# andabi/parallel-wavenet-vocoder

Hardware: AMD Instinct MI355X
Metric: audio samples/sec, 4-flow IAF generation (higher is better)
Workload: dtype f32 via 3-term split-fp16 MFMA (fp32 accumulate, fp32 storage)

## Files before the change

### parallel-wavenet-vocoder_amd/csrc/pwv_misc.hip

```cpp
#include "pwv_common.h"

#include <cstring>

namespace pwv {

static thread_local char g_err[512] = {0};
char* error_buffer() { return g_err; }
int set_error(int code, const char* fmt, ...) {
    va_list ap;
    va_start(ap, fmt);
    vsnprintf(g_err, sizeof(g_err), fmt, ap);
    va_end(ap);
    return code;
}

__global__ void causal_conv_kernel(const float* __restrict__ x, const float* __restrict__ f, float* __restrict__ y,
                                   int N, int T, int Cin, int Cout, int W, int d) {
    const int co4 = (Cout + 3) / 4;
    const long long idx = (long long)blockIdx.x * blockDim.x + threadIdx.x;
    const long long total = (long long)N * T * co4;
    if (idx >= total) return;
    const int c4 = (int)(idx % co4);
    const long long row = idx / co4;
    const int t = (int)(row % T);
// ... 56 lines not shown
        const int m = rt * 32 + j;
        const bool mvalid = m < M;
        const int mc = mvalid ? m : M - 1;
        float xb[KH4 * 4];
        const float* xr = x + (size_t)mc * K + h * kh;
        bool keep = true;
        if (conv_T > 0) {
            keep = h == 1 || (mc % conv_T) >= conv_d;
            xr = x + (size_t)(mc - ((h == 0 && keep) ? conv_d : 0)) * kh;
        }
#pragma unroll
        for (int g = 0; g < KH4; ++g) {
            f32x4 v = {0.f, 0.f, 0.f, 0.f};
            if (4 * g < kh && keep) v = *reinterpret_cast<const f32x4*>(xr + 4 * g);
#pragma unroll
            for (int e = 0; e < 4; ++e) xb[4 * g + e] = v[e];
        }
        f32x16 acc[4];
#pragma unroll
        for (int it = 0; it < 4; ++it)
#pragma unroll
            for (int r = 0; r < 16; ++r) {
                const int n = n0 + chan_of(it, r, h);
                acc[it][r] = (bias && n < Nout) ? bias[n] : 0.f;
            }
        f32x4 a[4];
#pragma unroll
        for (int it = 0; it < 4; ++it) a[it] = *reinterpret_cast<const f32x4*>(&lds[((it * KH4) * 64 + lane) * 4]);
#pragma unroll
        for (int g = 0; g < KH4; ++g) {
            if (4 * g < kh) {
                f32x4 nx[4] = {a[0], a[1], a[2], a[3]};
                if (g + 1 < KH4) {
#pragma unroll
                    for (int it = 0; it < 4; ++it)
                        nx[it] = *reinterpret_cast<const f32x4*>(&lds[((it * KH4 + g + 1) * 64 + lane) * 4]);
                }
                __builtin_amdgcn_sched_barrier(0);
#pragma unroll
                for (int e = 0; e < 4; ++e)
#pragma unroll
                    for (int it = 0; it < 4; ++it)
                        acc[it] = __builtin_amdgcn_mfma_f32_32x32x2f32(a[it][e], xb[4 * g + e], acc[it], 0, 0, 0);
                __builtin_amdgcn_sched_barrier(0);
#pragma unroll
                for (int it = 0; it < 4; ++it) a[it] = nx[it];
            }
        }
        if (mvalid) {
#pragma unroll
            for (int it = 0; it < 4; ++it)
#pragma unroll
                for (int q = 0; q < 4; ++q) {
                    const int n = n0 + 32 * it + 8 * q + 4 * h;
                    if (n < Nout) {
                        f32x4 v = {acc[it][q * 4], acc[it][q * 4 + 1], acc[it][q * 4 + 2], acc[it][q * 4 + 3]};
                        if (relu) {
#pragma unroll
                            for (int e = 0; e < 4; ++e) v[e] = fmaxf(v[e], 0.f);
                        }
                        *reinterpret_cast<f32x4*>(y + (size_t)m * Nout + n) = v;
                    }
                }
        }
    }
}

typedef float f32x2m __attribute__((ext_vector_type(2)));
__device__ __forceinline__ void split8m(const float (&x)[8], f16x8& hi, f16x8& lo) {
#pragma unroll
    for (int q = 0; q < 8; q += 2) {
        const f32x2m v = {x[q], x[q + 1]};
        const f16x2 h = __builtin_convertvector(v, f16x2);
        const f32x2m r = v - __builtin_convertvector(h, f32x2m);
        const f16x2 l = __builtin_convertvector(r, f16x2);
        hi[q] = h[0];
        hi[q + 1] = h[1];
        lo[q] = l[0];
        lo[q + 1] = l[1];
    }
}

template <int NS>
__global__ __launch_bounds__(256) void linear_split_kernel(const float* __restrict__ x, const float* __restrict__ w,
                                                           const float* __restrict__ bias, float* __restrict__ y, int M,
                                                           int K, int Nout, int relu) {
    __shared__ __attribute__((aligned(16))) f16x8 lds[2 * 4 * NS * 64];
    const int tid = threadIdx.x;
    const int lane = tid & 63;
    const int wave = __builtin_amdgcn_readfirstlane(tid >> 6);
    const int h = lane >> 5, j = lane & 31;
    const int n0 = blockIdx.y * 128;
    for (int item = tid; item < 128 * NS * 2; item += 256) {
        const int c = item & 127, sh = item >> 7, ss = sh >> 1, hh = sh & 1;
        float v[8];
#pragma unroll
        for (int q = 0; q < 8; ++q) {
            const int k = 16 * ss + 8 * hh + q;
            v[q] = (k < K && n0 + c < Nout) ? w[(size_t)k * Nout + n0 + c] : 0.f;
        }
        f16x8 hi, lo;
        split8m(v, hi, lo);
        const int unit = ((c >> 5) * NS + ss) * 64 + hh * 32 + (c & 31);
        lds[unit] = hi;
        lds[4 * NS * 64 + unit] = lo;
    }
    __syncthreads();
    const f16x8* AH = lds;
    const f16x8* AL = lds + 4 * NS * 64;
    const int row_tiles = (M + 31) / 32;
    for (int rt = blockIdx.x * 4 + wave; rt < row_tiles; rt += gridDim.x * 4) {
        const int m = rt * 32 + j;
        const bool mvalid = m < M;
        const int mc = mvalid ? m : M - 1;
        f16x8 bh[NS], bl[NS];
#pragma unroll
        for (int ss = 0; ss < NS; ++ss) {
            float v[8];
#pragma unroll
            for (int g = 0; g < 2; ++g) {
                const int k = 16 * ss + 8 * h + 4 * g;
                f32x4 t = {0.f, 0.f, 0.f, 0.f};
                if (k < K) t = *reinterpret_cast<const f32x4*>(x + (size_t)mc * K + k);
#pragma unroll
                for (int e = 0; e < 4; ++e) v[4 * g + e] = t[e];
            }
            split8m(v, bh[ss], bl[ss]);
        }
        f32x16 acc[4];
#pragma unroll
        for (int it = 0; it < 4; ++it) {
            const int n = n0 + 32 * it + j;
            const float bv = (bias && n < Nout) ? bias[n] : 0.f;
#pragma unroll
            for (int r = 0; r < 16; ++r) acc[it][r] = bv;
        }
#pragma unroll
        for (int ss = 0; ss < NS; ++ss) {
            f16x8 ah[4], al[4];
#pragma unroll
            for (int it = 0; it < 4; ++it) {
                ah[it] = AH[(it * NS + ss) * 64 + lane];
                al[it] = AL[(it * NS + ss) * 64 + lane];
            }
#pragma unroll
            for (int it = 0; it < 4; ++it) {
                acc[it] = __builtin_amdgcn_mfma_f32_32x32x16_f16(bh[ss], ah[it], acc[it], 0, 0, 0);
                acc[it] = __builtin_amdgcn_mfma_f32_32x32x16_f16(bl[ss], ah[it], acc[it], 0, 0, 0);
                acc[it] = __builtin_amdgcn_mfma_f32_32x32x16_f16(bh[ss], al[it], acc[it], 0, 0, 0);
            }
        }
#pragma unroll
        for (int it = 0; it < 4; ++it) {
            const int n = n0 + 32 * it + j;
#pragma unroll
            for (int r = 0; r < 16; ++r) {
                const int mr = rt * 32 + 8 * (r >> 2) + 4 * h + (r & 3);
                float v = acc[it][r];
                if (relu) v = fmaxf(v, 0.f);
                if (mr < M && n < Nout) __hip_atomic_store(&y[(size_t)mr * Nout + n], v, __ATOMIC_RELAXED, __HIP_MEMORY_SCOPE_AGENT);
            }
        }
    }
}

constexpr int kCtStride = 84;
__global__ __launch_bounds__(256) void cond_proj_kernel(const float* __restrict__ x0, const float* __restrict__ w0, int K0,
                                                        const float* __restrict__ w, const float* __restrict__ bias, float* __restrict__ y,
                                                        float* __restrict__ frames, int M, int K, int Nout, float limit, int* flag) {
    constexpr int NS = 5;
    __shared__ __attribute__((aligned(16))) f16x8 lds[2 * 4 * NS * 64];
    __shared__ __attribute__((aligned(16))) f16x8 lds0[2 * 4 * NS * 64];
    __shared__ __attribute__((aligned(16))) float ct[4][32 * kCtStride];
    const int tid = threadIdx.x;
    const int lane = tid & 63;
    const int wave = __builtin_amdgcn_readfirstlane(tid >> 6);
    const int h = lane >> 5, j = lane & 31;
    const int n0 = blockIdx.y * 128;
    for (int item = tid; item < 128 * NS * 2; item += 256) {
        const int c = item & 127, sh = item >> 7, ss = sh >> 1, hh = sh & 1;
        float v[8], v0[8];
#pragma unroll
        for (int q = 0; q < 8; ++q) {
            const int k = 16 * ss + 8 * hh + q;
            v[q] = (k < K && n0 + c < Nout) ? w[(size_t)k * Nout + n0 + c] : 0.f;
            v0[q] = (k < K0 && c < K) ? w0[(size_t)k * K + c] : 0.f;
        }
        f16x8 hi, lo;
        split8m(v, hi, lo);
        const int unit = ((c >> 5) * NS + ss) * 64 + hh * 32 + (c & 31);
        lds[unit] = hi;
        lds[4 * NS * 64 + unit] = lo;
        split8m(v0, hi, lo);
        lds0[unit] = hi;
        lds0[4 * NS * 64 + unit] = lo;
    }
    __syncthreads();
    const f16x8* AH = lds;
    const f16x8* AL = lds + 4 * NS * 64;
    const f16x8* A0H = lds0;
    const f16x8* A0L = lds0 + 4 * NS * 64;
    float* const ctw = ct[wave];
    const int row_tiles = (M + 31) / 32;
    for (int rt = blockIdx.x * 4 + wave; rt < row_tiles; rt += gridDim.x * 4) {
        const int m = rt * 32 + j;
        const bool mvalid = m < M;
        const int mc = mvalid ? m : M - 1;
        f16x8 bh[NS], bl[NS];
        bool bad = false;
#pragma unroll
        for (int ss = 0; ss < NS; ++ss) {
            float v[8];
#pragma unroll
            for (int g = 0; g < 2; ++g) {
                const int k = 16 * ss + 8 * h + 4 * g;
                f32x4 t = {0.f, 0.f, 0.f, 0.f};
                if (k < K0) t = *reinterpret_cast<const f32x4*>(x0 + (size_t)mc * K0 + k);
#pragma unroll
                for (int e = 0; e < 4; ++e) {
                    v[4 * g + e] = t[e];
                    bad = bad || !(fabsf(t[e]) <= limit);
                }
            }
            split8m(v, bh[ss], bl[ss]);
        }
        if (flag && bad) __hip_atomic_store(flag, 1, __ATOMIC_RELAXED, __HIP_MEMORY_SCOPE_SYSTEM);
        f32x16 acc0[3];
#pragma unroll
        for (int it = 0; it < 3; ++it)
#pragma unroll
            for (int r = 0; r < 16; ++r) acc0[it][r] = 0.f;
#pragma unroll
        for (int ss = 0; ss < NS; ++ss) {
            f16x8 ah[3], al[3];
#pragma unroll
            for (int it = 0; it < 3; ++it) {
                ah[it] = A0H[(it * NS + ss) * 64 + lane];
                al[it] = A0L[(it * NS + ss) * 64 + lane];
            }
#pragma unroll
            for (int it = 0; it < 3; ++it) {
                acc0[it] = __builtin_amdgcn_mfma_f32_32x32x16_f16(bh[ss], ah[it], acc0[it], 0, 0, 0);
                acc0[it] = __builtin_amdgcn_mfma_f32_32x32x16_f16(bl[ss], ah[it], acc0[it], 0, 0, 0);
                acc0[it] = __builtin_amdgcn_mfma_f32_32x32x16_f16(bh[ss], al[it], acc0[it], 0, 0, 0);
            }
        }
#pragma unroll
        for (int it = 0; it < 3; ++it) {
            const int n = 32 * it + j;
#pragma unroll
            for (int r = 0; r < 16; ++r) {
                const int ml = 8 * (r >> 2) + 4 * h + (r & 3);
                const float v = fmaxf(acc0[it][r], 0.f);
                if (n < K) {
                    ctw[ml * kCtStride + n] = v;
                    const int mr = rt * 32 + ml;
                    if (frames && blockIdx.y == 0 && mr < M) __hip_atomic_store(&frames[(size_t)mr * K + n], v, __ATOMIC_RELAXED, __HIP_MEMORY_SCOPE_AGENT);
                }
            }
        }
        asm volatile("s_waitcnt lgkmcnt(0)" ::: "memory");
#pragma unroll
        for (int ss = 0; ss < NS; ++ss) {
            float v[8];
#pragma unroll
            for (int g = 0; g < 2; ++g) {
                const int k = 16 * ss + 8 * h + 4 * g;
                f32x4 t = {0.f, 0.f, 0.f, 0.f};
                if (k < K) t = *reinterpret_cast<const f32x4*>(&ctw[j * kCtStride + k]);
#pragma unroll
                for (int e = 0; e < 4; ++e) v[4 * g + e] = t[e];
            }
            split8m(v, bh[ss], bl[ss]);
        }
        asm volatile("s_waitcnt lgkmcnt(0)" ::: "memory");
        f32x16 acc[4];
#pragma unroll
        for (int it = 0; it < 4; ++it) {
            const int n = n0 + 32 * it + j;
            const float bv = (bias && n < Nout) ? bias[n] : 0.f;
#pragma unroll
            for (int r = 0; r < 16; ++r) acc[it][r] = bv;
        }
#pragma unroll
        for (int ss = 0; ss < NS; ++ss) {
            f16x8 ah[4], al[4];
#pragma unroll
            for (int it = 0; it < 4; ++it) {
                ah[it] = AH[(it * NS + ss) * 64 + lane];
                al[it] = AL[(it * NS + ss) * 64 + lane];
            }
#pragma unroll
            for (int it = 0; it < 4; ++it) {
                acc[it] = __builtin_amdgcn_mfma_f32_32x32x16_f16(bh[ss], ah[it], acc[it], 0, 0, 0);
                acc[it] = __builtin_amdgcn_mfma_f32_32x32x16_f16(bl[ss], ah[it], acc[it], 0, 0, 0);
                acc[it] = __builtin_amdgcn_mfma_f32_32x32x16_f16(bh[ss], al[it], acc[it], 0, 0, 0);
            }
        }
#pragma unroll
        for (int it = 0; it < 4; ++it) {
            const int n = n0 + 32 * it + j;
#pragma unroll
            for (int r = 0; r < 16; ++r) {
                const int mr = rt * 32 + 8 * (r >> 2) + 4 * h + (r & 3);
                if (mr < M && n < Nout) __hip_atomic_store(&y[(size_t)mr * Nout + n], acc[it][r], __ATOMIC_RELAXED, __HIP_MEMORY_SCOPE_AGENT);
            }
        }
    }
}

__global__ void upsample_repeat_kernel(const float* __restrict__ frames, float* __restrict__ out, int N, int t_mel,
                                       int C4, int T, int hop, int offset) {
    const long long idx = (long long)blockIdx.x * blockDim.x + threadIdx.x;
    const long long total = (long long)N * T * C4;
    if (idx >= total) return;
    const int c = (int)(idx % C4);
    const long long row = idx / C4;
    const int t = (int)(row % T);
    const int n = (int)(row / T);
    int fr = (t + offset) / hop;
    fr = fr < t_mel ? fr : t_mel - 1;
    reinterpret_cast<f32x4*>(out)[idx] = reinterpret_cast<const f32x4*>(frames)[((size_t)n * t_mel + fr) * C4 + c];
}

__global__ void crop_time_kernel(const float* __restrict__ in, float* __restrict__ out, int N, int T_in, int C4,
                                 int T_out, int offset) {
    const long long idx = (long long)blockIdx.x * blockDim.x + threadIdx.x;
    const long long total = (long long)N * T_out * C4;
    if (idx >= total) return;
    const int c = (int)(idx % C4);
    const long long row = idx / C4;
    const int t = (int)(row % T_out);
    const int n = (int)(row / T_out);
    reinterpret_cast<f32x4*>(out)[idx] = reinterpret_cast<const f32x4*>(in)[((size_t)n * T_in + t + offset) * C4 + c];
}

__device__ __forceinline__ float logistic_of_counter(unsigned long long seed, unsigned long long counter) {
    unsigned long long s = seed * 0x9E3779B97F4A7C15ull + counter;
    s += 0x9E3779B97F4A7C15ull;
    s = (s ^ (s >> 30)) * 0xBF58476D1CE4E5B9ull;
    s = (s ^ (s >> 27)) * 0x94D049BB133111EBull;
    s = s ^ (s >> 31);
    const float u = ((float)(unsigned)(s >> 41) + 0.5f) * (1.0f / 8388608.0f);
    return logf(u) - log1pf(-u);
}

__global__ void logistic_noise_kernel(float* __restrict__ z, long long n, unsigned long long seed,
                                      unsigned long long offset) {
    const long long i = (long long)blockIdx.x * blockDim.x + threadIdx.x;
    if (i >= n) return;
    z[i] = logistic_of_counter(seed, (unsigned long long)i + offset);
}

__global__ void logistic_noise_stream_kernel(float* __restrict__ z, long long n, unsigned long long* state) {
    __shared__ unsigned long long sh[3];
    if (threadIdx.x == 0) {
        sh[0] = __hip_atomic_load(&state[0], __ATOMIC_RELAXED, __HIP_MEMORY_SCOPE_AGENT);
        sh[1] = __hip_atomic_load(&state[1], __ATOMIC_RELAXED, __HIP_MEMORY_SCOPE_AGENT);
        sh[2] = __hip_atomic_load(&state[3], __ATOMIC_RELAXED, __HIP_MEMORY_SCOPE_AGENT);
    }
    __syncthreads();
    const unsigned long long seed = sh[0], offset = sh[1];
    const bool skip = sh[2] != 0;
    const long long i = (long long)blockIdx.x * blockDim.x + threadIdx.x;
    if (i < n && !skip) z[i] = logistic_of_counter(seed, (unsigned long long)i + offset);
    __syncthreads();
    if (threadIdx.x == 0) {
        const unsigned long long done = __hip_atomic_fetch_add(&state[2], 1ull, __ATOMIC_ACQ_REL, __HIP_MEMORY_SCOPE_AGENT);
        if (done == (unsigned long long)gridDim.x - 1ull) {
            if (!skip) __hip_atomic_store(&state[1], offset + (unsigned long long)n, __ATOMIC_RELAXED, __HIP_MEMORY_SCOPE_AGENT);
            __hip_atomic_store(&state[2], 0ull, __ATOMIC_RELAXED, __HIP_MEMORY_SCOPE_AGENT);
        }
    }
}

__global__ __launch_bounds__(256) void logistic_noise_packed_kernel(float* __restrict__ z, const int* __restrict__ cu_rows,
                                                                    const unsigned long long* __restrict__ streams, int n, long long rows) {
    const long long r = (long long)blockIdx.x * blockDim.x + threadIdx.x;
    if (r >= rows) return;
    int lo = 0, hi = n - 1;
    while (lo < hi) {
        const int mid = (lo + hi + 1) >> 1;
        if ((long long)cu_rows[mid] <= r) lo = mid;
        else hi = mid - 1;
    }
    const unsigned long long seed = streams[2 * lo], offset = streams[2 * lo + 1];
    z[r] = logistic_of_counter(seed, offset + (unsigned long long)(r - (long long)cu_rows[lo]));
}

struct FrontParams {
    const float* z;
    const float* s;
    const float* b;
    float* x_out;
    const float* filt[PWV_MAX_NETS];
    float* h[PWV_MAX_NETS];
    int sb_stride, G, N, T, W, R;
};

constexpr int kFrontMaxTaps = 8;
constexpr int kFrontMaxFilt = 2048;

__global__ __launch_bounds__(256) void iaf_front_kernel(const FrontParams p) {
    __shared__ __attribute__((aligned(16))) float fl[kFrontMaxFilt];
    const int g = blockIdx.y;
    if (p.G > 0) {
        for (int i = threadIdx.x; i < p.W * p.R; i += 256) fl[i] = p.filt[g][i];
        __syncthreads();
    }
    const unsigned rows = (unsigned)p.N * (unsigned)p.T;
    const unsigned row = blockIdx.x * 256u + threadIdx.x;
    if (row >= rows) return;
    const unsigned t = row % (unsigned)p.T;
    auto xval = [&](unsigned rr) -> float {
        const float zv = p.z[rr];
        return p.s ? fmaf(zv, p.s[(size_t)rr * p.sb_stride], p.b[(size_t)rr * p.sb_stride]) : zv;
    };
    const float xcur = xval(row);
    float xv[kFrontMaxTaps];
#pragma unroll
    for (int k = 0; k < kFrontMaxTaps; ++k) {
        const unsigned shift = (unsigned)(p.W - 1 - k);
        xv[k] = k + 1 == p.W ? xcur : ((k < p.W && shift <= t) ? xval(row - shift) : 0.f);
    }
    if (g == 0 && p.x_out) p.x_out[row] = xcur;
    if (p.G == 0) return;
    float* out = p.h[g] + (size_t)(row >> 5) * (32u * p.R) + (row & 31u) * 4u;
    const int r4 = p.R / 4;
    for (int q = 0; q < r4; ++q) {
        f32x4 acc = {0.f, 0.f, 0.f, 0.f};
#pragma unroll
        for (int k = 0; k < kFrontMaxTaps; ++k) {
            if (k < p.W) {
                const f32x4 w = *reinterpret_cast<const f32x4*>(&fl[k * p.R + 4 * q]);
#pragma unroll
                for (int e = 0; e < 4; ++e) acc[e] = fmaf(xv[k], w[e], acc[e]);
            }
        }
        *reinterpret_cast<f32x4*>(out + q * 128) = acc;
    }
}

template <bool TO_TILE>
__global__ void tile32_kernel(const float* __restrict__ in, float* __restrict__ out, unsigned rows, unsigned c4) {
    const unsigned idx = blockIdx.x * blockDim.x + threadIdx.x;
    const unsigned row = (idx / (32u * c4)) * 32u + (idx & 31u), quad = (idx >> 5) % c4;
    if (row >= rows) return;
    const size_t lin = (size_t)row * c4 * 4 + quad * 4, til = (size_t)(row >> 5) * (128u * c4) + quad * 128u + (row & 31u) * 4u;
// ... 27 lines not shown
    return PWV_OK;
}

int pwv_status_words_alloc(int** words) {
    PWV_CHECK_ARG(words, "pwv_status_words_alloc: NULL argument");
    int* w = nullptr;
    PWV_CHECK_HIP(hipHostMalloc((void**)&w, 2 * sizeof(int), hipHostMallocMapped | hipHostMallocPortable));
    w[0] = w[1] = 0;
    *words = w;
    return PWV_OK;
}

int pwv_status_words_free(int* words) {
    if (words) PWV_CHECK_HIP(hipHostFree(words));
    return PWV_OK;
}

int pwv_range_check_f32(const float* x, int64_t n, float limit, int* flag, pwv_stream_t stream) {
    PWV_CHECK_ARG(x && flag && n >= 0, "pwv_range_check_f32: bad arguments");
    if (n == 0) return PWV_OK;
    hipLaunchKernelGGL(range_check_kernel, dim3(blocks_for(n, 256)), dim3(256), 0, (hipStream_t)stream, x, (long long)n, limit, flag);
    PWV_CHECK_HIP(hipGetLastError());
    return PWV_OK;
}
int pwv_device_cus(void) {
    const int c = device_cus();
    return c > 0 ? c : set_error(PWV_EHIP, "no HIP device available");
}

static int launch_linear(const float* x, const float* w, const float* bias, float* y, int M, int K, int Nout, int relu, int conv_T, int conv_d,
                         pwv_stream_t stream);

int pwv_causal_conv_f32(const float* x, const float* filt, float* y, int N, int T, int Cin, int Cout, int W,
                        int dilation, pwv_stream_t stream) {
    PWV_CHECK_ARG(x && filt && y, "pwv_causal_conv_f32: NULL pointer");
    PWV_CHECK_ARG(N >= 0 && T >= 0 && Cin >= 1 && Cout >= 1 && W >= 1 && dilation >= 1,
                  "pwv_causal_conv_f32: bad shape N=%d T=%d Cin=%d Cout=%d W=%d d=%d", N, T, Cin, Cout, W, dilation);
    PWV_CHECK_ARG(x != y, "pwv_causal_conv_f32: in-place not supported");
    const long long total = (long long)N * T * ((Cout + 3) / 4);
    if (total == 0) return PWV_OK;
    if ((long long)N * T < (1ll << 31) && Cout % 4 == 0 && x != y) {
        if (W == 1 && Cin % 8 == 0 && Cin <= 128) return launch_linear(x, filt, nullptr, y, N * T, Cin, Cout, 0, 0, 0, stream);
        if (W == 2 && Cin % 4 == 0 && Cin <= 64) return launch_linear(x, filt, nullptr, y, N * T, 2 * Cin, Cout, 0, T, dilation, stream);
    }
    hipLaunchKernelGGL(causal_conv_kernel, dim3(blocks_for(total, 256)), dim3(256), 0, (hipStream_t)stream, x, filt, y,
                       N, T, Cin, Cout, W, dilation);
    PWV_CHECK_HIP(hipGetLastError());
    return PWV_OK;
}

int pwv_linear_f32(const float* x, const float* w, const float* bias, float* y, int M, int K, int Nout, int relu,
                   pwv_stream_t stream) {
    PWV_CHECK_ARG(x && w && y, "pwv_linear_f32: NULL pointer");
    PWV_CHECK_ARG(M >= 0 && K >= 8 && K % 8 == 0 && K <= 128, "pwv_linear_f32: K must be a multiple of 8 in [8,128], got %d", K);
    PWV_CHECK_ARG(Nout >= 4 && Nout % 4 == 0, "pwv_linear_f32: Nout must be a multiple of 4, got %d", Nout);
    return launch_linear(x, w, bias, y, M, K, Nout, relu, 0, 0, stream);
}

static int launch_linear(const float* x, const float* w, const float* bias, float* y, int M, int K, int Nout, int relu, int conv_T, int conv_d,
                         pwv_stream_t stream) {
    if (M == 0) return PWV_OK;
    const int kh = K / 2;
    const unsigned gy = (unsigned)((Nout + 127) / 128);
    unsigned gx = (unsigned)((M + 127) / 128);
    const unsigned cap = (1024u + gy - 1) / gy;
    if (gx > cap) gx = cap;
    if (gx < 1) gx = 1;
    dim3 grid(gx, gy), block(256);
    hipStream_t s = (hipStream_t)stream;
    if (kh <= 32)
        hipLaunchKernelGGL((linear_kernel<8>), grid, block, 0, s, x, w, bias, y, M, K, Nout, relu, conv_T, conv_d);
    else if (kh <= 40)
        hipLaunchKernelGGL((linear_kernel<10>), grid, block, 0, s, x, w, bias, y, M, K, Nout, relu, conv_T, conv_d);
    else
        hipLaunchKernelGGL((linear_kernel<16>), grid, block, 0, s, x, w, bias, y, M, K, Nout, relu, conv_T, conv_d);
    PWV_CHECK_HIP(hipGetLastError());
    return PWV_OK;
}

int pwv_linear_split_f32(const float* x, const float* w, const float* bias, float* y, int M, int K, int Nout, int relu,
                         pwv_stream_t stream) {
    PWV_CHECK_ARG(x && w && y, "pwv_linear_split_f32: NULL pointer");
    PWV_CHECK_ARG(M >= 0 && K >= 8 && K % 8 == 0 && K <= 128, "pwv_linear_split_f32: K must be a multiple of 8 in [8,128], got %d", K);
    PWV_CHECK_ARG(Nout >= 4 && Nout % 4 == 0, "pwv_linear_split_f32: Nout must be a multiple of 4, got %d", Nout);
    if (M == 0) return PWV_OK;
    const unsigned gy = (unsigned)((Nout + 127) / 128);
    unsigned gx = (unsigned)((M + 127) / 128);
    const unsigned cap = (1024u + gy - 1) / gy;
    if (gx > cap) gx = cap;
    if (gx < 1) gx = 1;
    dim3 grid(gx, gy), block(256);
    hipStream_t s = (hipStream_t)stream;
    if (K <= 64)
        hipLaunchKernelGGL((linear_split_kernel<4>), grid, block, 0, s, x, w, bias, y, M, K, Nout, relu);
    else if (K <= 80)
        hipLaunchKernelGGL((linear_split_kernel<5>), grid, block, 0, s, x, w, bias, y, M, K, Nout, relu);
    else
        hipLaunchKernelGGL((linear_split_kernel<8>), grid, block, 0, s, x, w, bias, y, M, K, Nout, relu);
    PWV_CHECK_HIP(hipGetLastError());
    return PWV_OK;
}

int pwv_cond_project_f32(const float* mel, const float* dense, int n_mels, const float* bank_w, const float* bank_b, float* frames,
                         float* P, int M, int C, int Nout, float limit, int* range_flag, pwv_stream_t stream) {
    PWV_CHECK_ARG(mel && dense && bank_w && P, "pwv_cond_project_f32: NULL pointer");
    PWV_CHECK_ARG(M >= 0 && n_mels >= 8 && n_mels % 8 == 0 && n_mels <= 80 && C >= 8 && C % 8 == 0 && C <= 80,
                  "pwv_cond_project_f32: n_mels and C must be multiples of 8 in [8, 80], got %d / %d", n_mels, C);
    PWV_CHECK_ARG(Nout >= 4 && Nout % 4 == 0, "pwv_cond_project_f32: Nout must be a multiple of 4, got %d", Nout);
    if (M == 0) return PWV_OK;
    const unsigned gy = (unsigned)((Nout + 127) / 128);
    unsigned gx = (unsigned)((M + 127) / 128);
    const unsigned cap = (1024u + gy - 1) / gy;
    if (gx > cap) gx = cap;
    if (gx < 1) gx = 1;
    hipLaunchKernelGGL(cond_proj_kernel, dim3(gx, gy), dim3(256), 0, (hipStream_t)stream, mel, dense, n_mels, bank_w, bank_b, P, frames, M, C, Nout,
                       range_flag ? limit : 3.0e38f, range_flag);
    PWV_CHECK_HIP(hipGetLastError());
    return PWV_OK;
}

int pwv_upsample_repeat_f32(const float* frames, float* out, int N, int t_mel, int C, int T, int hop, int offset,
                            pwv_stream_t stream) {
    PWV_CHECK_ARG(frames && out, "pwv_upsample_repeat_f32: NULL pointer");
    PWV_CHECK_ARG(N >= 0 && t_mel >= 1 && C >= 4 && C % 4 == 0 && T >= 0 && hop >= 1 && offset >= 0,
                  "pwv_upsample_repeat_f32: bad shape (C must be a multiple of 4)");
    PWV_CHECK_ARG(T == 0 || (T - 1 + offset) / hop < t_mel, "pwv_upsample_repeat_f32: T=%d needs more than t_mel=%d frames", T, t_mel);
    const long long total = (long long)N * T * (C / 4);
    if (total == 0) return PWV_OK;
    hipLaunchKernelGGL(upsample_repeat_kernel, dim3(blocks_for(total, 256)), dim3(256), 0, (hipStream_t)stream, frames,
                       out, N, t_mel, C / 4, T, hop, offset);
    PWV_CHECK_HIP(hipGetLastError());
    return PWV_OK;
}

int pwv_crop_time_f32(const float* in, float* out, int N, int T_in, int C, int T_out, int offset, pwv_stream_t stream) {
    PWV_CHECK_ARG(in && out, "pwv_crop_time_f32: NULL pointer");
    PWV_CHECK_ARG(C >= 4 && C % 4 == 0 && offset >= 0 && T_out >= 0 && offset + T_out <= T_in,
                  "pwv_crop_time_f32: bad crop (T_in=%d T_out=%d offset=%d C=%d)", T_in, T_out, offset, C);
    const long long total = (long long)N * T_out * (C / 4);
    if (total == 0) return PWV_OK;
    hipLaunchKernelGGL(crop_time_kernel, dim3(blocks_for(total, 256)), dim3(256), 0, (hipStream_t)stream, in, out, N,
                       T_in, C / 4, T_out, offset);
    PWV_CHECK_HIP(hipGetLastError());
    return PWV_OK;
}

int pwv_logistic_noise_f32(float* z, int64_t n, uint64_t seed, uint64_t offset, pwv_stream_t stream) {
    PWV_CHECK_ARG(z && n >= 0, "pwv_logistic_noise_f32: bad arguments");
    if (n == 0) return PWV_OK;
    hipLaunchKernelGGL(logistic_noise_kernel, dim3(blocks_for(n, 256)), dim3(256), 0, (hipStream_t)stream, z,
                       (long long)n, (unsigned long long)seed, (unsigned long long)offset);
    PWV_CHECK_HIP(hipGetLastError());
    return PWV_OK;
}

int pwv_logistic_noise_stream_f32(float* z, int64_t n, uint64_t* state, pwv_stream_t stream) {
    PWV_CHECK_ARG(z && state && n >= 0, "pwv_logistic_noise_stream_f32: bad arguments");
    if (n == 0) return PWV_OK;
    hipLaunchKernelGGL(logistic_noise_stream_kernel, dim3(blocks_for(n, 256)), dim3(256), 0, (hipStream_t)stream, z, (long long)n,
                       (unsigned long long*)state);
    PWV_CHECK_HIP(hipGetLastError());
    return PWV_OK;
}

int pwv_logistic_noise_packed_f32(float* z, const int32_t* cu_rows, const uint64_t* streams, int32_t n, int64_t rows,
                                  pwv_stream_t stream) {
    PWV_CHECK_ARG(z && cu_rows && streams, "pwv_logistic_noise_packed_f32: NULL pointer");
    PWV_CHECK_ARG(n >= 1 && rows >= 0 && rows <= 0x7fffffffLL, "pwv_logistic_noise_packed_f32: bad n=%d / rows=%lld (cu_rows is int32)",
                  (int)n, (long long)rows);
    if (rows == 0) return PWV_OK;
    hipLaunchKernelGGL(logistic_noise_packed_kernel, dim3(blocks_for(rows, 256)), dim3(256), 0, (hipStream_t)stream, z,
                       (const int*)cu_rows, (const unsigned long long*)streams, (int)n, (long long)rows);
    PWV_CHECK_HIP(hipGetLastError());
    return PWV_OK;
}

int pwv_iaf_front_f32(const float* z, const float* s, const float* b, int sb_stride, float* x_out, int G,
                      const float* const* filt, float* const* h, int N, int T, int W, int R, pwv_stream_t stream) {
    PWV_CHECK_ARG(z, "pwv_iaf_front_f32: z is NULL");
    PWV_CHECK_ARG((s == nullptr) == (b == nullptr), "pwv_iaf_front_f32: s and b must both be set or both NULL");
    PWV_CHECK_ARG(G >= 0 && G <= PWV_MAX_NETS, "pwv_iaf_front_f32: G=%d out of range", G);
    PWV_CHECK_ARG(N >= 1 && T >= 1 && W >= 1, "pwv_iaf_front_f32: bad N/T/W");
    PWV_CHECK_ARG(G == 0 || (R >= 4 && R % 4 == 0), "pwv_iaf_front_f32: R must be a multiple of 4");
    PWV_CHECK_ARG(G > 0 || x_out, "pwv_iaf_front_f32: nothing to do");
    PWV_CHECK_ARG(sb_stride >= 1 || !s, "pwv_iaf_front_f32: sb_stride must be >= 1");
    FrontParams p{};
    p.z = z;
    p.s = s;
    p.b = b;
    p.x_out = x_out;
    p.sb_stride = sb_stride;
    p.G = G;
    p.N = N;
    p.T = T;
    p.W = W;
    p.R = R;
    for (int g = 0; g < G; ++g) {
        PWV_CHECK_ARG(filt && h && filt[g] && h[g], "pwv_iaf_front_f32: NULL filter / output for net %d", g);
        p.filt[g] = filt[g];
        p.h[g] = h[g];
    }
    PWV_CHECK_ARG((long long)N * T < (1ll << 31) - 256, "pwv_iaf_front_f32: N*T must stay below 2^31");
    PWV_CHECK_ARG(G == 0 || (W <= kFrontMaxTaps && W * R <= kFrontMaxFilt),
                  "pwv_iaf_front_f32: filter width %d / %d channels not supported (W <= %d, W*R <= %d)", W, R, kFrontMaxTaps, kFrontMaxFilt);
    PWV_CHECK_ARG(W <= kFrontMaxTaps, "pwv_iaf_front_f32: W must be <= %d", kFrontMaxTaps);
    hipLaunchKernelGGL(iaf_front_kernel, dim3(blocks_for((long long)N * T, 256), G > 0 ? G : 1), dim3(256), 0, (hipStream_t)stream, p);
    PWV_CHECK_HIP(hipGetLastError());
    return PWV_OK;
}

size_t pwv_tile32_floats(int64_t rows, int C) { return rows > 0 && C > 0 ? (size_t)((rows + 31) / 32) * 32 * (size_t)C : 0; }

static int tile32_convert(bool to_tile, const float* in, float* out, int64_t rows, int C, pwv_stream_t stream) {
    PWV_CHECK_ARG(in && out && in != out, "pwv tile32 conversion: NULL or aliased buffers");
    PWV_CHECK_ARG(rows >= 0 && C >= 4 && C % 4 == 0, "pwv tile32 conversion: C must be a positive multiple of 4");
    const long long total = (rows + 31) / 32 * 32 * (C / 4);
    PWV_CHECK_ARG(total < (1ll << 31), "pwv tile32 conversion: rows*C/4 must stay below 2^31");
    if (total == 0) return PWV_OK;
    if (to_tile)
        hipLaunchKernelGGL(tile32_kernel<true>, dim3(blocks_for(total, 256)), dim3(256), 0, (hipStream_t)stream, in, out,
                           (unsigned)rows, (unsigned)(C / 4));
    else
        hipLaunchKernelGGL(tile32_kernel<false>, dim3(blocks_for(total, 256)), dim3(256), 0, (hipStream_t)stream, in, out,
                           (unsigned)rows, (unsigned)(C / 4));
    PWV_CHECK_HIP(hipGetLastError());
    return PWV_OK;
}

int pwv_rows_to_tile32_f32(const float* in, float* out, int64_t rows, int C, pwv_stream_t stream) {
    return tile32_convert(true, in, out, rows, C, stream);
}

int pwv_tile32_to_rows_f32(const float* in, float* out, int64_t rows, int C, pwv_stream_t stream) {
    return tile32_convert(false, in, out, rows, C, stream);
}

}
```

### parallel-wavenet-vocoder_amd/engine.py

```python
from __future__ import annotations

import ctypes
import numbers
import os
import threading
import weakref
from ctypes import c_void_p
from typing import Dict, List, NamedTuple, Optional, Sequence, Tuple

import torch

from . import _lib
from ._lib import StackArgs, check

PRECISIONS = {'f32': _lib.PREC_F32, 'f16x3': _lib.PREC_F16X3, 'f16': _lib.PREC_F16}
DEFAULT_PRECISION = os.environ.get('PWV_PRECISION', 'f16x3')

EVENT_LOG = None

TWO_STREAMS = os.environ.get('PWV_TWO_STREAMS', '1') != '0'
FUSE_FIRST = True
FUSE_HEAD = True
FUSE_TAIL = os.environ.get('PWV_FUSE_TAIL', '1') != '0'
HOIST_P = True
# ... 644 lines not shown
    G, L, prec = len(nets), plans[0].n_layers, plans[0].precision
    net0 = nets[0]
    stride = plans[0].layer_floats

    if not path.first_fused:
        la = _layer_args(net0, plans, projs, row_stride, cond_geom, bufs, 0, 0, 2, x)
        la.out_mode = _lib.OUT_RESIDUAL
        check(lib.pwv_wavenet_layer_f32(ctypes.byref(la), s), 'pwv_wavenet_layer_f32')

    Q = net0.out_channels
    affine_fused = bool(path.tail and affine is not None and ((G == 2 and Q == 1) or (G == 1 and Q == 2)))
    for j0, pa in path.runs:
        for g in range(G):
            pa.x_ring[g] = bufs[g][0].data_ptr()
            pa.packed_layers[g] = plans[g].packed_layers.data_ptr() + 4 * stride * j0
            pa.proj[g] = projs[g].data_ptr() + 4 * 128 * j0
        pa.ring_stride, pa.proj_row_stride = bufs[0][0].numel(), row_stride
        if j0 == 0:
            _set_x_first(pa, plans, x, x_limit)
        if geom is not None:
            geom.set_args(pa)
        tail_here = path.tail and pa is path.runs[-1][1]
        if stream_hist is not None:
            sa, row_off = stream_hist
            layers = list(range(j0, j0 + pa.n_layers)) + ([L - 1] if tail_here else [])
            hist_offs = [(ctypes.c_size_t * len(layers))(*[max(int(row_off[g][j]), 0) for j in layers]) for g in range(G)]
            pa.hist = ctypes.addressof(sa)
            for g in range(G):
                pa.hist_row_off[g] = hist_offs[g]
        wkey = (bufs[0][0].device, torch.cuda.current_stream().cuda_stream)
        ws = _persist_ws.get(wkey)
        if ws is None or ws.numel() < pa.workspace_bytes:
            ws = _persist_ws[wkey] = torch.zeros((max(pa.workspace_bytes, 1 << 16),), dtype=torch.uint8, device=bufs[0][0].device)
        pa.workspace, pa.workspace_clean = ws.data_ptr(), 1
        pa.status = persist_status_ptr()
        if tail_here:
            for g in range(G):
                pa.tail_layer[g] = plans[g].packed_layers.data_ptr() + 4 * stride * (L - 1)
                pa.tail_head[g] = plans[g].packed_head.data_ptr()
                pa.tail_out[g] = outs[g].data_ptr()
            if affine_fused:
                pa.affine_x, pa.affine_out = affine[0].data_ptr(), affine[1].data_ptr()
        ev = None
        if EVENT_LOG is not None:
            ev = (torch.cuda.Event(enable_timing=True), torch.cuda.Event(enable_timing=True))
            ev[0].record()
        if PERSIST_ARGS_HOOK is not None:
            PERSIST_ARGS_HOOK(pa)
        check(lib.pwv_wavenet_stack_persist_f32(ctypes.byref(pa), s), 'pwv_wavenet_stack_persist_f32')
        if ev is not None:
            ev[1].record()
            EVENT_LOG.append(('persist', ev[0], ev[1], G, pa.n_layers, 1 if j0 == 0 else 0, 1 if tail_here else 0,
                              int(lib.pwv_persist_short_input(ctypes.byref(pa))),
                              1 if stream_hist is not None else 0))
    if path.tail:
        return affine_fused
    last = path.runs[-1][1]
    out_slot = (last.n_layers - 1 + last.ring_rotation) % 3
    spare = (out_slot + 1) % 3

    la = _layer_args(net0, plans, projs, row_stride, cond_geom, bufs, L - 1, out_slot, spare, x)
    la.out_mode = _lib.OUT_GATED
    fuse_head = head_fusable(prec)
    if fuse_head:
        for g in range(G):
            la.head_packed[g] = plans[g].packed_head.data_ptr()
            la.head_out[g] = outs[g].data_ptr()
        la.head_q = Q
    check(lib.pwv_wavenet_layer_f32(ctypes.byref(la), s), 'pwv_wavenet_layer_f32')
    if not fuse_head:
        ha = _lib.HeadArgs()
        ha.G, ha.N, ha.T, ha.Q = G, x.shape[0], x.shape[1], Q
        for g in range(G):
            ha.in_[g], ha.packed[g], ha.out[g] = bufs[g][spare].data_ptr(), plans[g].packed_head.data_ptr(), outs[g].data_ptr()
        ha.in_mode, ha.precision = _lib.HEAD_IN_GATED, prec
        check(lib.pwv_wavenet_head_f32(ctypes.byref(ha), s), 'pwv_wavenet_head_f32')
    return False


_bank_cache = {}


FUSE_PROLOGUE = os.environ.get('PWV_FUSE_PROLOGUE', '1') != '0'
FUSE_PROLOGUE_MAX_OUTPUTS = 1 << 21


def _projection_bank(nets: Sequence, channels: int, prec: int):
    for _ in range(2):
        versions = [net.store.version for net in nets]
        plans = []
        for net in nets:
            if not getattr(net, 'fused_supported', None) or channels != net.condition_channels:
                continue
            if not net.fused_supported(_FrameShape(channels)):
                continue
            p = get_plan(net, 'frames', prec)
            if prec == _lib.PREC_F16X3 and not (p.f16x3_ok and p.x_limit > 0):
                continue
            if all(p is not q for q in plans):
                plans.append(p)
        if versions == [net.store.version for net in nets]:
            break
    if len(plans) < 2:
        return None
    key = tuple(id(p) for p in plans)
    hit = _bank_cache.get(key)
    if hit is None:
        if len(_bank_cache) >= 8:
            _bank_cache.clear()
        offs, total = [], 0
        for p in plans:
            offs.append(total)
            total += p.proj_w.shape[1]
        hit = (plans, torch.cat([p.proj_w for p in plans], dim=1).contiguous(), torch.cat([p.proj_b for p in plans]).contiguous(), offs)
        _bank_cache[key] = hit
    return hit


class _FrameShape(RepeatedCondition):

    def __init__(self, channels):
        self.frames = torch.empty((0, 1, channels))
        self.hop = self.offset = self.length = 0


def project_all(nets: Sequence, cond, precision: Optional[str] = None) -> None:
    if not HOIST_P or not isinstance(cond, RepeatedCondition) or not nets or getattr(cond, 'proj_bank', None) is not None:
        return
    prec = PRECISIONS[precision or DEFAULT_PRECISION]
    bank = _projection_bank(nets, cond.frames.shape[2], prec)
    if bank is None:
        return
    plans, w_all, b_all, offs = bank
    n, frames, c = cond.frames.shape
    f2d = _require_cuda_f32(cond.frames, 'frames').reshape(n * frames, c)
    p_all = linear_op(f2d, w_all, b_all, relu=False, precision=precision or DEFAULT_PRECISION)
    cond.proj_bank = {id(p): p_all[:, o:o + p.proj_w.shape[1]] for p, o in zip(plans, offs)}


def repeat_condition_with_projections(nets: Sequence, melspec: torch.Tensor, dense: torch.Tensor, hop: int, length: int,
                                      precision: Optional[str], mel_limit: Optional[float]):
    name = precision or DEFAULT_PRECISION
    if not (FUSE_PROLOGUE and HOIST_P) or name == 'f32' or not nets:
        return None
    n, t_mel, n_mels = melspec.shape
    c = dense.shape[1]
    if n_mels % 8 or c % 8 or n_mels > 80 or c > 80:
        return None
    bank = _projection_bank(nets, c, PRECISIONS[name])
    if bank is None:
        return None
    plans, w_all, b_all, offs = bank
    m = n * t_mel
    if m * w_all.shape[1] > FUSE_PROLOGUE_MAX_OUTPUTS:
        return None
    frames = torch.empty((n, t_mel, c), dtype=torch.float32, device=melspec.device)
    p_all = torch.empty((m, w_all.shape[1]), dtype=torch.float32, device=melspec.device)
    flag = range_flag_ptr() if (name == 'f16x3' and mel_limit is not None) else None
    if flag is not None:
        _log_range('mel', melspec, mel_limit)
    check(_lib.lib().pwv_cond_project_f32(_ptr(melspec), _ptr(dense), n_mels, _ptr(w_all), _ptr(b_all), _ptr(frames), _ptr(p_all), m, c,
                                          w_all.shape[1], float(mel_limit or 0.0), flag, _stream()), 'pwv_cond_project_f32')
    cond = RepeatedCondition(frames, hop, hop // 2, length)
    cond.proj_bank = {id(p): p_all[:, o:o + p.proj_w.shape[1]] for p, o in zip(plans, offs)}
    return cond


# ... 648 lines not shown
```

Baseline: 60.60 million.

## Vectorize weight staging and output stores, regroup cond projection, grid-stride noise

Weight staging now loads float4 columns before splitting to fp16 hi/lo, and output tiles are transposed through an LDS slab so they leave as 128-bit buffer stores instead of scalar atomic stores. The conditioning projection kernel reuses one LDS plane for the dense weights, the c tiles and the bank weights. Each block now walks a group of column blocks, so the first projection is done once per row tile instead of once per column block, and launch bounds allow two blocks per CU. The noise kernel becomes grid-stride with vectorized stores, and the fused-prologue output cap is effectively removed. The cost is extra LDS round trips and syncs, plus more work per block when groups are large.

```diff
diff --git a/parallel-wavenet-vocoder_amd/csrc/pwv_misc.hip b/parallel-wavenet-vocoder_amd/csrc/pwv_misc.hip
--- a/parallel-wavenet-vocoder_amd/csrc/pwv_misc.hip
+++ b/parallel-wavenet-vocoder_amd/csrc/pwv_misc.hip
@@ -162,29 +162,95 @@
 }
 
 template <int NS>
+__device__ __forceinline__ void stage_split_block(f16x8* __restrict__ lds, const float* __restrict__ w, int K, int ncols, int n0, int tid,
+                                                  bool vec) {
+    for (int item = tid; item < 32 * NS * 2; item += 256) {
+        const int c = (item & 31) * 4, sh = item >> 5, ss = sh >> 1, hh = sh & 1;
+        const bool inside = 16 * ss + 8 * hh < K && n0 + c < ncols;
+        const float* src = w + (inside ? (size_t)(16 * ss + 8 * hh) * ncols + n0 + c : 0);
+        const size_t step = inside ? (size_t)ncols : 0;
+        f32x4 t[8];
+        if (vec) {
+#pragma unroll
+            for (int q = 0; q < 8; ++q) t[q] = *reinterpret_cast<const f32x4*>(src + q * step);
+        } else {
+#pragma unroll
+            for (int q = 0; q < 8; ++q) t[q] = f32x4{src[q * step], src[q * step + 1], src[q * step + 2], src[q * step + 3]};
+        }
+        if (!inside) {
+#pragma unroll
+            for (int q = 0; q < 8; ++q) t[q] = f32x4{0.f, 0.f, 0.f, 0.f};
+        }
+#pragma unroll
+        for (int e = 0; e < 4; ++e) {
+            float v[8];
+#pragma unroll
+            for (int q = 0; q < 8; ++q) v[q] = t[q][e];
+            f16x8 hi, lo;
+            split8m(v, hi, lo);
+            const int unit = ((c >> 5) * NS + ss) * 64 + hh * 32 + ((c & 31) + e);
+            lds[unit] = hi;
+            lds[4 * NS * 64 + unit] = lo;
+        }
+    }
+}
+
+constexpr int kSlabStride = 136;
+typedef unsigned u32x4m __attribute__((ext_vector_type(4)));
+__device__ __forceinline__ void store_tile_rows(float* slab, const f32x16 (&acc)[4], int relu, float* __restrict__ y, int M, int Nout,
+                                                int rt, int n0, int lane, bool y_vec) {
+    const int h = lane >> 5, j = lane & 31;
+    const int rows = M - rt * 32 < 32 ? M - rt * 32 : 32;
+    float* const ybase = y + (size_t)rt * 32 * Nout;
+    const unsigned long long a = (unsigned long long)ybase;
+    const unsigned lo = __builtin_amdgcn_readfirstlane((unsigned)a), hi = __builtin_amdgcn_readfirstlane((unsigned)(a >> 32));
+    const unsigned bytes = __builtin_amdgcn_readfirstlane((unsigned)rows * (unsigned)Nout * 4u);
+    const __amdgpu_buffer_rsrc_t rs = __builtin_amdgcn_make_buffer_rsrc((void*)(((unsigned long long)hi << 32) | lo), 0, bytes, 0x00020000);
+    const int col = n0 + 4 * j;
+#pragma unroll
+    for (int rg = 0; rg < 4; ++rg) {
+#pragma unroll
+        for (int it = 0; it < 4; ++it)
+#pragma unroll
+            for (int q = 0; q < 4; ++q) {
+                float v = acc[it][4 * rg + q];
+                if (relu) v = fmaxf(v, 0.f);
+                slab[(4 * h + q) * kSlabStride + 32 * it + j] = v;
+            }
+        asm volatile("s_waitcnt lgkmcnt(0)" ::: "memory");
+#pragma unroll
+        for (int p = 0; p < 4; ++p) {
+            const int rl = 8 * rg + 2 * p + h;
+            const f32x4 v = *reinterpret_cast<const f32x4*>(&slab[(2 * p + h) * kSlabStride + 4 * j]);
+            if (rl < rows && col < Nout) {
+                if (y_vec) {
+                    __builtin_amdgcn_raw_buffer_store_b128(__builtin_bit_cast(u32x4m, v), rs, (rl * Nout + col) * 4, 0, 16 );
+                } else {
+#pragma unroll
+                    for (int e = 0; e < 4; ++e)
+                        __hip_atomic_store(&ybase[(size_t)rl * Nout + col + e], v[e], __ATOMIC_RELAXED, __HIP_MEMORY_SCOPE_AGENT);
+                }
+            }
+        }
+        asm volatile("s_waitcnt lgkmcnt(0)" ::: "memory");
+    }
+}
+
+__device__ __forceinline__ bool aligned16(const void* p) { return ((unsigned long long)p & 15ull) == 0; }
+
+template <int NS>
 __global__ __launch_bounds__(256) void linear_split_kernel(const float* __restrict__ x, const float* __restrict__ w,
                                                            const float* __restrict__ bias, float* __restrict__ y, int M,
                                                            int K, int Nout, int relu) {
     __shared__ __attribute__((aligned(16))) f16x8 lds[2 * 4 * NS * 64];
+    __shared__ __attribute__((aligned(16))) float slab[4][8 * kSlabStride];
     const int tid = threadIdx.x;
     const int lane = tid & 63;
     const int wave = __builtin_amdgcn_readfirstlane(tid >> 6);
     const int h = lane >> 5, j = lane & 31;
     const int n0 = blockIdx.y * 128;
-    for (int item = tid; item < 128 * NS * 2; item += 256) {
-        const int c = item & 127, sh = item >> 7, ss = sh >> 1, hh = sh & 1;
-        float v[8];
-#pragma unroll
-        for (int q = 0; q < 8; ++q) {
-            const int k = 16 * ss + 8 * hh + q;
-            v[q] = (k < K && n0 + c < Nout) ? w[(size_t)k * Nout + n0 + c] : 0.f;
-        }
-        f16x8 hi, lo;
-        split8m(v, hi, lo);
-        const int unit = ((c >> 5) * NS + ss) * 64 + hh * 32 + (c & 31);
-        lds[unit] = hi;
-        lds[4 * NS * 64 + unit] = lo;
-    }
+    const bool y_vec = aligned16(y);
+    stage_split_block<NS>(lds, w, K, Nout, n0, tid, aligned16(w));
     __syncthreads();
     const f16x8* AH = lds;
     const f16x8* AL = lds + 4 * NS * 64;
@@ -230,63 +296,34 @@
                 acc[it] = __builtin_amdgcn_mfma_f32_32x32x16_f16(bh[ss], al[it], acc[it], 0, 0, 0);
             }
         }
-#pragma unroll
-        for (int it = 0; it < 4; ++it) {
-            const int n = n0 + 32 * it + j;
-#pragma unroll
-            for (int r = 0; r < 16; ++r) {
-                const int mr = rt * 32 + 8 * (r >> 2) + 4 * h + (r & 3);
-                float v = acc[it][r];
-                if (relu) v = fmaxf(v, 0.f);
-                if (mr < M && n < Nout) __hip_atomic_store(&y[(size_t)mr * Nout + n], v, __ATOMIC_RELAXED, __HIP_MEMORY_SCOPE_AGENT);
-            }
-        }
-    }
-}
-
-constexpr int kCtStride = 84;
-__global__ __launch_bounds__(256) void cond_proj_kernel(const float* __restrict__ x0, const float* __restrict__ w0, int K0,
+        store_tile_rows(slab[wave], acc, relu, y, M, Nout, rt, n0, lane, y_vec);
+    }
+}
+
+constexpr int kCtStride = 80;
+__global__ __launch_bounds__(256, 2) void cond_proj_kernel(const float* __restrict__ x0, const float* __restrict__ w0, int K0,
                                                         const float* __restrict__ w, const float* __restrict__ bias, float* __restrict__ y,
-                                                        float* __restrict__ frames, int M, int K, int Nout, float limit, int* flag) {
+                                                        float* __restrict__ frames, int M, int K, int Nout, float limit, int* flag, int group) {
     constexpr int NS = 5;
     __shared__ __attribute__((aligned(16))) f16x8 lds[2 * 4 * NS * 64];
-    __shared__ __attribute__((aligned(16))) f16x8 lds0[2 * 4 * NS * 64];
-    __shared__ __attribute__((aligned(16))) float ct[4][32 * kCtStride];
+    __shared__ __attribute__((aligned(16))) float slab[4][8 * kSlabStride];
+    static_assert(4 * 32 * kCtStride * sizeof(float) <= sizeof(lds), "the c tiles live in the fragment planes");
     const int tid = threadIdx.x;
     const int lane = tid & 63;
     const int wave = __builtin_amdgcn_readfirstlane(tid >> 6);
     const int h = lane >> 5, j = lane & 31;
-    const int n0 = blockIdx.y * 128;
-    for (int item = tid; item < 128 * NS * 2; item += 256) {
-        const int c = item & 127, sh = item >> 7, ss = sh >> 1, hh = sh & 1;
-        float v[8], v0[8];
-#pragma unroll
-        for (int q = 0; q < 8; ++q) {
-            const int k = 16 * ss + 8 * hh + q;
-            v[q] = (k < K && n0 + c < Nout) ? w[(size_t)k * Nout + n0 + c] : 0.f;
-            v0[q] = (k < K0 && c < K) ? w0[(size_t)k * K + c] : 0.f;
-        }
-        f16x8 hi, lo;
-        split8m(v, hi, lo);
-        const int unit = ((c >> 5) * NS + ss) * 64 + hh * 32 + (c & 31);
-        lds[unit] = hi;
-        lds[4 * NS * 64 + unit] = lo;
-        split8m(v0, hi, lo);
-        lds0[unit] = hi;
-        lds0[4 * NS * 64 + unit] = lo;
-    }
-    __syncthreads();
     const f16x8* AH = lds;
     const f16x8* AL = lds + 4 * NS * 64;
-    const f16x8* A0H = lds0;
-    const f16x8* A0L = lds0 + 4 * NS * 64;
-    float* const ctw = ct[wave];
-    const int row_tiles = (M + 31) / 32;
-    for (int rt = blockIdx.x * 4 + wave; rt < row_tiles; rt += gridDim.x * 4) {
+    const int rt = blockIdx.x * 4 + wave;
+    const bool active = rt < (M + 31) / 32;
+    const bool y_vec = aligned16(y), w_vec = aligned16(w);
+    stage_split_block<NS>(lds, w0, K0, K, 0, tid, aligned16(w0));
+    __syncthreads();
+    f16x8 bh[NS], bl[NS];
+    f32x16 acc0[3];
+    if (active) {
         const int m = rt * 32 + j;
-        const bool mvalid = m < M;
-        const int mc = mvalid ? m : M - 1;
-        f16x8 bh[NS], bl[NS];
+        const int mc = m < M ? m : M - 1;
         bool bad = false;
 #pragma unroll
         for (int ss = 0; ss < NS; ++ss) {
@@ -305,7 +342,6 @@
             split8m(v, bh[ss], bl[ss]);
         }
         if (flag && bad) __hip_atomic_store(flag, 1, __ATOMIC_RELAXED, __HIP_MEMORY_SCOPE_SYSTEM);
-        f32x16 acc0[3];
 #pragma unroll
         for (int it = 0; it < 3; ++it)
 #pragma unroll
@@ -315,8 +351,8 @@
             f16x8 ah[3], al[3];
 #pragma unroll
             for (int it = 0; it < 3; ++it) {
-                ah[it] = A0H[(it * NS + ss) * 64 + lane];
-                al[it] = A0L[(it * NS + ss) * 64 + lane];
+                ah[it] = AH[(it * NS + ss) * 64 + lane];
+                al[it] = AL[(it * NS + ss) * 64 + lane];
             }
 #pragma unroll
             for (int it = 0; it < 3; ++it) {
@@ -325,6 +361,10 @@
                 acc0[it] = __builtin_amdgcn_mfma_f32_32x32x16_f16(bh[ss], al[it], acc0[it], 0, 0, 0);
             }
         }
+    }
+    __syncthreads();
+    if (active) {
+        float* const ctw = reinterpret_cast<float*>(lds) + wave * (32 * kCtStride);
 #pragma unroll
         for (int it = 0; it < 3; ++it) {
             const int n = 32 * it + j;
@@ -354,6 +394,15 @@
             split8m(v, bh[ss], bl[ss]);
         }
         asm volatile("s_waitcnt lgkmcnt(0)" ::: "memory");
+    }
+    const int col_blocks = (Nout + 127) / 128;
+    const int cb_end = (int)(blockIdx.y + 1) * group < col_blocks ? (int)(blockIdx.y + 1) * group : col_blocks;
+    for (int cb = blockIdx.y * group; cb < cb_end; ++cb) {
+        const int n0 = cb * 128;
+        __syncthreads();
+        stage_split_block<NS>(lds, w, K, Nout, n0, tid, w_vec);
+        __syncthreads();
+        if (!active) continue;
         f32x16 acc[4];
 #pragma unroll
         for (int it = 0; it < 4; ++it) {
@@ -377,15 +426,7 @@
                 acc[it] = __builtin_amdgcn_mfma_f32_32x32x16_f16(bh[ss], al[it], acc[it], 0, 0, 0);
             }
         }
-#pragma unroll
-        for (int it = 0; it < 4; ++it) {
-            const int n = n0 + 32 * it + j;
-#pragma unroll
-            for (int r = 0; r < 16; ++r) {
-                const int mr = rt * 32 + 8 * (r >> 2) + 4 * h + (r & 3);
-                if (mr < M && n < Nout) __hip_atomic_store(&y[(size_t)mr * Nout + n], acc[it][r], __ATOMIC_RELAXED, __HIP_MEMORY_SCOPE_AGENT);
-            }
-        }
+        store_tile_rows(slab[wave], acc, 0, y, M, Nout, rt, n0, lane, y_vec);
     }
 }
 
@@ -432,7 +473,7 @@
     z[i] = logistic_of_counter(seed, (unsigned long long)i + offset);
 }
 
-__global__ void logistic_noise_stream_kernel(float* __restrict__ z, long long n, unsigned long long* state) {
+__global__ __launch_bounds__(256) void logistic_noise_stream_kernel(float* __restrict__ z, long long n, unsigned long long* state) {
     __shared__ unsigned long long sh[3];
     if (threadIdx.x == 0) {
         sh[0] = __hip_atomic_load(&state[0], __ATOMIC_RELAXED, __HIP_MEMORY_SCOPE_AGENT);
@@ -442,8 +483,19 @@
     __syncthreads();
     const unsigned long long seed = sh[0], offset = sh[1];
     const bool skip = sh[2] != 0;
-    const long long i = (long long)blockIdx.x * blockDim.x + threadIdx.x;
-    if (i < n && !skip) z[i] = logistic_of_counter(seed, (unsigned long long)i + offset);
+    if (!skip) {
+        const long long stride = (long long)gridDim.x * blockDim.x;
+        const long long t = (long long)blockIdx.x * blockDim.x + threadIdx.x;
+        const long long quads = ((unsigned long long)z & 15ull) == 0 ? n / 4 : 0;
+        for (long long q = t; q < quads; q += stride) {
+            const unsigned long long c = (unsigned long long)(4 * q) + offset;
+            f32x4 v;
+#pragma unroll
+            for (int e = 0; e < 4; ++e) v[e] = logistic_of_counter(seed, c + (unsigned long long)e);
+            *reinterpret_cast<f32x4*>(z + 4 * q) = v;
+        }
+        for (long long i = 4 * quads + t; i < n; i += stride) z[i] = logistic_of_counter(seed, (unsigned long long)i + offset);
+    }
     __syncthreads();
     if (threadIdx.x == 0) {
         const unsigned long long done = __hip_atomic_fetch_add(&state[2], 1ull, __ATOMIC_ACQ_REL, __HIP_MEMORY_SCOPE_AGENT);
@@ -637,7 +689,7 @@
                          pwv_stream_t stream) {
     PWV_CHECK_ARG(x && w && y, "pwv_linear_split_f32: NULL pointer");
     PWV_CHECK_ARG(M >= 0 && K >= 8 && K % 8 == 0 && K <= 128, "pwv_linear_split_f32: K must be a multiple of 8 in [8,128], got %d", K);
-    PWV_CHECK_ARG(Nout >= 4 && Nout % 4 == 0, "pwv_linear_split_f32: Nout must be a multiple of 4, got %d", Nout);
+    PWV_CHECK_ARG(Nout >= 4 && Nout % 4 == 0 && Nout <= (1 << 24), "pwv_linear_split_f32: Nout must be a multiple of 4 up to 2^24, got %d", Nout);
     if (M == 0) return PWV_OK;
     const unsigned gy = (unsigned)((Nout + 127) / 128);
     unsigned gx = (unsigned)((M + 127) / 128);
@@ -663,13 +715,15 @@
                   "pwv_cond_project_f32: n_mels and C must be multiples of 8 in [8, 80], got %d / %d", n_mels, C);
     PWV_CHECK_ARG(Nout >= 4 && Nout % 4 == 0, "pwv_cond_project_f32: Nout must be a multiple of 4, got %d", Nout);
     if (M == 0) return PWV_OK;
-    const unsigned gy = (unsigned)((Nout + 127) / 128);
-    unsigned gx = (unsigned)((M + 127) / 128);
-    const unsigned cap = (1024u + gy - 1) / gy;
-    if (gx > cap) gx = cap;
-    if (gx < 1) gx = 1;
-    hipLaunchKernelGGL(cond_proj_kernel, dim3(gx, gy), dim3(256), 0, (hipStream_t)stream, mel, dense, n_mels, bank_w, bank_b, P, frames, M, C, Nout,
-                       range_flag ? limit : 3.0e38f, range_flag);
+    PWV_CHECK_ARG(Nout <= (1 << 24), "pwv_cond_project_f32: Nout must not exceed 2^24, got %d", Nout);
+    const long long col_blocks = (Nout + 127) / 128, row_chunks = (M + 127) / 128;
+    const int cus = device_cus();
+    const long long slots = 2 * (long long)(cus > 0 ? cus : 256);
+    long long group = (row_chunks * col_blocks + slots - 1) / slots;
+    group = group < 1 ? 1 : (group > 8 ? 8 : group);
+    const unsigned gy = (unsigned)((col_blocks + group - 1) / group);
+    hipLaunchKernelGGL(cond_proj_kernel, dim3((unsigned)row_chunks, gy), dim3(256), 0, (hipStream_t)stream, mel, dense, n_mels, bank_w, bank_b, P, frames, M, C, Nout,
+                       range_flag ? limit : 3.0e38f, range_flag, (int)group);
     PWV_CHECK_HIP(hipGetLastError());
     return PWV_OK;
 }
@@ -712,7 +766,9 @@
 int pwv_logistic_noise_stream_f32(float* z, int64_t n, uint64_t* state, pwv_stream_t stream) {
     PWV_CHECK_ARG(z && state && n >= 0, "pwv_logistic_noise_stream_f32: bad arguments");
     if (n == 0) return PWV_OK;
-    hipLaunchKernelGGL(logistic_noise_stream_kernel, dim3(blocks_for(n, 256)), dim3(256), 0, (hipStream_t)stream, z, (long long)n,
+    const int cus = device_cus();
+    const long long want = (n + 1023) / 1024, cap = cus > 0 ? cus : 256;
+    hipLaunchKernelGGL(logistic_noise_stream_kernel, dim3((unsigned)(want < cap ? want : cap)), dim3(256), 0, (hipStream_t)stream, z, (long long)n,
                        (unsigned long long*)state);
     PWV_CHECK_HIP(hipGetLastError());
     return PWV_OK;
diff --git a/parallel-wavenet-vocoder_amd/engine.py b/parallel-wavenet-vocoder_amd/engine.py
--- a/parallel-wavenet-vocoder_amd/engine.py
+++ b/parallel-wavenet-vocoder_amd/engine.py
@@ -750,7 +750,7 @@
 
 
 FUSE_PROLOGUE = os.environ.get('PWV_FUSE_PROLOGUE', '1') != '0'
-FUSE_PROLOGUE_MAX_OUTPUTS = 1 << 21
+FUSE_PROLOGUE_MAX_OUTPUTS = 1 << 40
 
 
 def _projection_bank(nets: Sequence, channels: int, prec: int):
```

Result: no change. 60.86 million (median of 6 runs) (+0.4%).
